# speechcatcher-asr/speechcatcher

Hardware: AMD Instinct MI355X
Metric: concurrent real-time streams (audio-seconds/s), de_xl dims, 640 ms (10240-sample) chunk steps, beam 10 CTC+attention (higher is better)
Workload: dtype f32

## Files before the change

### speechcatcher_amd/csrc/common.h

```cpp
#pragma once
#include <hip/hip_runtime.h>
#include <stdint.h>
#include <stdio.h>
#include <math.h>

#include "../../include/scasr.h"

#define SC_LOGZERO (-10000000000.0f)

void sc_set_error(const char *fmt, ...);

const char *sc_hook(const char *name);

__attribute__((visibility("hidden"))) int allow_large_lds(const void *fn, size_t need, size_t max_bytes, const char *what);

#define SC_CHECK_ARG(cond, msg)      \
  do {                               \
    if (!(cond)) {                   \
      sc_set_error("%s: %s", __func__, msg); \
      return SC_ERR_ARG;             \
    }                                \
  } while (0)

#define SC_CHECK_LAUNCH()                                              \
  do {                                                                 \
    hipError_t e__ = hipGetLastError();                                \
    if (e__ != hipSuccess) {                                           \
      sc_set_error("%s: launch failed: %s", __func__, hipGetErrorString(e__)); \
      return SC_ERR_LAUNCH;                                            \
    }                                                                  \
  } while (0)

__host__ __device__ static inline int cdiv(int a, int b) { return (a + b - 1) / b; }

#define SC_TRY(call) do { rc = (call); if (rc != SC_OK) return rc; } while (0)

struct ProfScope {
  bool on; hipEvent_t a, b; hipStream_t st;
  ProfScope(bool on_, hipEvent_t a_, hipEvent_t b_, hipStream_t st_) : on(on_), a(a_), b(b_), st(st_) {}
  ProfScope(const ProfScope &) = delete;
  __attribute__((visibility("hidden"))) ~ProfScope() {
    if (on) { (void)hipEventDestroy(a); (void)hipEventDestroy(b); }
  }
};
ProfScope sc_prof_begin(hipStream_t st);
void sc_prof_end(ProfScope &p, int kind, double flops, double bytes);

int sc_decode_step_form(const sc_search *sb);
int sc_gemm_colblocks(const float *A, const int32_t *a_rows, int lda, const float *W, const float *bias, float *C,
                      const int32_t *c_rows, int ldc, int M, int N, int K, int ncb, long cb_stride, int flags, void *stream);

int sc_dec_layer_hpw(const sc_search &sb);
int sc_dec_layer_stream_form(const sc_search &sb);
int sc_dec_layer_split_ffn(const sc_search &sb);

int sc_launch_reduce_ln_proj(const float *part, int npart, int part_M, const float *b2, const float *Xin, float *Xout,
                             const int32_t *rows, int M, int D, const float *ln_g, const float *ln_b, float ln_eps,
                             float *XN, const float *Wq, const float *bq, float *Q, int N, hipStream_t st,
                             int by_row = 0, int half_mode = 0);

struct ScHandoff { const int32_t *blkinfo; int R; float *state; int layer; };
int sc_ffn_ln_handoff(const float *XN, int M, int D, int F, const void *W1, const float *b1, const void *W2, const float *b2,
                      float *X, int w_form, const ScHandoff &ho, void *stream);

template <int CTRL>
__device__ __forceinline__ float dpp_mov(float v) {
  return __int_as_float(__builtin_amdgcn_update_dpp(0, __float_as_int(v), CTRL, 0xF, 0xF, true));
}
#define SC_DPP_XOR1 0xB1
#define SC_DPP_XOR2 0x4E
#define SC_DPP_HALF_MIRROR 0x141
#define SC_DPP_ROR4 0x124
#define SC_DPP_ROR8 0x128
#define SC_DPP_ROW_MIRROR 0x140

template <int LPR>
__device__ __forceinline__ float group_sum(float v) {
  v += dpp_mov<SC_DPP_XOR1>(v);
  v += dpp_mov<SC_DPP_XOR2>(v);
  if (LPR >= 8) v += dpp_mov<SC_DPP_HALF_MIRROR>(v);
  if (LPR == 16) v += dpp_mov<SC_DPP_ROW_MIRROR>(v);
  return v;
}

__device__ __forceinline__ float sc_lane(float v, int lane) {
  return __int_as_float(__builtin_amdgcn_readlane(__float_as_int(v), lane));
}
__device__ __forceinline__ float wave_max(float v) {
  v = fmaxf(v, dpp_mov<SC_DPP_XOR1>(v));
  v = fmaxf(v, dpp_mov<SC_DPP_XOR2>(v));
  v = fmaxf(v, dpp_mov<SC_DPP_HALF_MIRROR>(v));
  v = fmaxf(v, dpp_mov<SC_DPP_ROW_MIRROR>(v));
  return fmaxf(fmaxf(sc_lane(v, 0), sc_lane(v, 16)), fmaxf(sc_lane(v, 32), sc_lane(v, 48)));
}
__device__ __forceinline__ float wave_sum(float v) {
  v += dpp_mov<SC_DPP_XOR1>(v);
  v += dpp_mov<SC_DPP_XOR2>(v);
  v += dpp_mov<SC_DPP_HALF_MIRROR>(v);
  v += dpp_mov<SC_DPP_ROW_MIRROR>(v);
  return (sc_lane(v, 0) + sc_lane(v, 16)) + (sc_lane(v, 32) + sc_lane(v, 48));
}

#define SC_LOG2E 1.4426950408889634f
#define SC_LN2 0.6931471805599453f
__device__ __forceinline__ float sc_exp_neg(float x) {
  return __builtin_amdgcn_exp2f(x * SC_LOG2E);
}
__device__ __forceinline__ float sc_max_raw(float a, float b) {
  float m;
  asm("v_max_f32 %0, %1, %2" : "=v"(m) : "v"(a), "v"(b));
  return m;
}
__device__ __forceinline__ float lse2(float a, float b) {
  const float m = sc_max_raw(a, b);
  return m + SC_LN2 * __builtin_amdgcn_logf(1.f + sc_exp_neg(-fabsf(a - b)));
}

__device__ __forceinline__ float4 sc_add4(const float4 &a, const float4 &b) {
  return make_float4(a.x + b.x, a.y + b.y, a.z + b.z, a.w + b.w);
}
__device__ __forceinline__ float4 sc_tree4(const float4 &a, const float4 &b, const float4 &c, const float4 &d) {
  return sc_add4(sc_add4(a, b), sc_add4(c, d));
}
__device__ __forceinline__ float4 sc_tree8(const float4 (&v)[8]) {
  return sc_add4(sc_tree4(v[0], v[1], v[2], v[3]), sc_tree4(v[4], v[5], v[6], v[7]));
}
__device__ __forceinline__ float sc_tree8f(const float (&v)[8]) {
  return ((v[0] + v[1]) + (v[2] + v[3])) + ((v[4] + v[5]) + (v[6] + v[7]));
}
__device__ __forceinline__ float4 sc_seq4(const float4 &a, const float4 &b, const float4 &c, const float4 &d) {
  return sc_add4(sc_add4(sc_add4(a, b), c), d);
// ... 63 lines not shown
```

### speechcatcher_amd/csrc/search.hip

```cpp
#include "common.h"
#include "attn.h"
#include <mutex>
#include <unordered_map>

#define CTRL(s, f) sb.ctrl[(s) * 8 + (f)]
#define SC_CTC_T(s) (CTRL(s, SC_C_TCTC) > 0 ? CTRL(s, SC_C_TCTC) : CTRL(s, SC_C_T))

#define YSEQ(pp, s, h) (sb.yseq + (((long)(pp) * sb.S + (s)) * sb.W + (h)) * sb.LCAP)
#define XPOS(pp, s, h) (sb.xpos + (((long)(pp) * sb.S + (s)) * sb.W + (h)) * sb.LCAP)
#define ANC(pp, s) (sb.anc + ((long)(pp) * sb.S + (s)) * sb.LCAP * sb.W)
#define CTCR(pp, s) (sb.ctc_r + ((long)(pp) * sb.S + (s)) * sb.TCAP * 2 * sb.W)
#define CTCRS(pp, s) (sb.ctc_rs + ((long)(pp) * sb.S + (s)) * sb.TCAP * sb.W)

__global__ void ctc_extend_state_kernel(sc_search sb) {
  const int s = blockIdx.x, h = threadIdx.x;
  if (!CTRL(s, SC_C_ACTIVE) || !CTRL(s, SC_C_HAS)) return;
  const int T = CTRL(s, SC_C_T), told = CTRL(s, SC_C_TOLD), nh = CTRL(s, SC_C_NHYP);
  if (h >= nh || told >= T) return;
  float *r = CTCR(CTRL(s, SC_C_CUR), s);
  float *rs = CTCRS(CTRL(s, SC_C_CUR), s);
  const float *x = sb.ctcx + (long)s * sb.TCAP * sb.V;
  const int t0 = told < 1 ? 1 : told;
  float rb = r[((long)(t0 - 1) * 2 + 1) * sb.W + h];
  for (int t = t0; t < T; ++t) {
// ... 1069 lines not shown
          dst_rs[(long)t * W + i] = lse2(SC_LOGZERO, SC_LOGZERO);
        }
        if (start - 1 < t1) {
          dst[((long)(start - 1) * 2) * W + i] = r_n;
          dst[((long)(start - 1) * 2 + 1) * W + i] = r_b;
          dst_rs[(long)(start - 1) * W + i] = lse2(r_n, r_b);
        }
        t_lo = start;
      } else {
        r_n = ck[((long)(j - 1) * 2) * WK + e];
        r_b = ck[((long)(j - 1) * 2 + 1) * WK + e];
        t_lo = t0;
      }
      t_hi = t1;
    }
    if (t_lo >= t_hi) continue;
    float cum = 0.f;
    if (!has)
      for (int t = 0; t < t_lo; ++t) cum += xblk[t];
    for (int tb = t_lo & ~(SC_CTC_CK - 1); tb < t_hi; tb += SC_CTC_CK) {
      float xc[SC_CTC_CK], xb[SC_CTC_CK], pn[SC_CTC_CK], pb[SC_CTC_CK];
#pragma unroll
      for (int q = 0; q < SC_CTC_CK / 4; ++q) {
        const int t4 = min(tb + 4 * q, tct - 4);
        const float4 c4 = *reinterpret_cast<const float4 *>(xcol + t4), b4 = *reinterpret_cast<const float4 *>(xblk + t4);
        xc[4 * q] = c4.x; xc[4 * q + 1] = c4.y; xc[4 * q + 2] = c4.z; xc[4 * q + 3] = c4.w;
        xb[4 * q] = b4.x; xb[4 * q + 1] = b4.y; xb[4 * q + 2] = b4.z; xb[4 * q + 3] = b4.w;
      }
#pragma unroll
      for (int q = 0; q < SC_CTC_CK; ++q) {
        const int tp = min(max(tb + q - 1, 0), T - 1);
        pn[q] = has ? rsp[(long)tp * W + h] : 0.f;
        pb[q] = has ? rp[((long)tp * 2 + 1) * W + h] : 0.f;
      }
#pragma unroll
      for (int q = 0; q < SC_CTC_CK; ++q) {
        const int t = tb + q;
        if (t >= t_lo && t < t_hi) {
          float phi;
          ctc_frame(r_n, r_b, has ? pn[q] : cum, has ? pb[q] : cum, same, xc[q], xb[q], phi);
          dst[((long)t * 2) * W + i] = r_n;
          dst[((long)t * 2 + 1) * W + i] = r_b;
          dst_rs[(long)t * W + i] = lse2(r_n, r_b);
          if (!has) cum += xb[q];
        }
      }
    }
  }
}

extern "C" int sc_ctc_gather_state_split(const sc_search *sbp, int split_min, void *stream) {
  SC_CHECK_ARG(sbp, "null");
  SC_CHECK_ARG(sbp->ctcxT && sbp->tct >= 4, "the state rebuild needs the column-major table copy (sc_search.ctcxT)");
  int gx = cdiv(ctc_tck(sbp->TCAP) * sbp->W, 256);
  if (gx > 16) gx = 16;
  const int eff = ctc_split_min_ok(sbp->TCAP, split_min), last = scan_split_last(sbp);
  if (last >= 0 && last != eff) {
    sc_set_error("sc_ctc_gather_state_split: the last prefix scan of this batch ran with split_min = %d, the rebuild was asked for %d - "
                 "streams split over T leave segment states, not checkpoints: pass the scan's value (sc_ctc_gather_state() = 0)", last, eff);
    return SC_ERR_ARG;
  }
  ctc_gather_state_kernel<<<dim3(gx, sbp->S), 256, 0, (hipStream_t)stream>>>(*sbp, eff);
  SC_CHECK_LAUNCH();
  return SC_OK;
}

extern "C" int sc_ctc_gather_state(const sc_search *sbp, void *stream) { return sc_ctc_gather_state_split(sbp, 0, stream); }

static bool dec_fused_ok(const sc_search &sb) {
  if (const char *e = sc_hook("SC_DEC_FUSED"))
    return atoi(e) != 0 && sc_dec_layer_fused_supported(sb.d, sb.H, sb.W, sb.F) && sb.ph1 && sb.out_w_q;
  if (const char *e = sc_hook("SC_FUSED_MAX"))
    if ((sb.rowmap ? sb.n_rows : sb.S * sb.W) > atoi(e) && sc_dec_layer_hpw(sb) < 2) return false;
  return sc_dec_layer_fused_supported(sb.d, sb.H, sb.W, sb.F) && sb.ph1 && sb.ph2 && sb.ffn_part &&
         sb.max_ffn_part >= 1 && sb.out_w_q && sb.V % sb.d == 0 && sb.layers && sb.layers[0].wqkv_pp &&
         sb.layers[0].wq_pp && sb.layers[0].wo_pp && sb.layers[0].w1_p;
}

int sc_decode_step_form(const sc_search *sbp) { return dec_fused_ok(*sbp) ? (sc_dec_layer_stream_form(*sbp) ? 2 : 1) : 0; }

extern "C" int sc_decode_step(const sc_search *sbp, void *stream) { return sc_decode_step_ex(sbp, 0, stream); }

extern "C" int sc_decode_step_ex(const sc_search *sbp, int scan_split_min, void *stream) {
  SC_CHECK_ARG(sbp, "null");
  const sc_search &sb = *sbp;
  const int n = sb.rowmap ? sb.n_rows : sb.S * sb.W;
  int rc;
  if (dec_fused_ok(sb) && sc_dec_layer_stream_form(sb)) {
    float *xa = sb.dx, *xb = sb.dxn;
    int npart = 0;
    for (int li = 0; li < sb.n_layers; ++li) {
      SC_TRY(sc_dec_layer_stream(sbp, li, xa, xb, sb.dq, sb.ffn_part, npart, stream));
      SC_TRY(sc_dec_layer_ffn_xn(sbp, li, sb.dq, sb.ffn_part, sb.max_ffn_part, &npart, stream));
      float *t = xa; xa = xb; xb = t;
    }
    SC_TRY(sc_dec_output_logits(sbp, xa, xb, sb.ffn_part, npart, stream));
  } else if (dec_fused_ok(sb)) {
    float *xa = sb.dx, *xb = sb.dxn;
    int npart = 0;
    for (int li = 0; li < sb.n_layers; ++li) {
      SC_TRY(sc_dec_layer_self(sbp, li, xa, xb, sb.ffn_part, npart, stream));
      SC_TRY(sc_dec_layer_cross(sbp, li, xb, xa, stream));
      if (sc_dec_layer_split_ffn(sb)) {
        SC_TRY(sc_dec_layer_reduce_ln(sbp, li, xa, xb, sb.dq, stream));
        SC_TRY(sc_dec_layer_ffn_xn(sbp, li, sb.dq, sb.ffn_part, sb.max_ffn_part, &npart, stream));
      } else
      SC_TRY(sc_dec_layer_ffn(sbp, li, xa, xb, sb.ffn_part, sb.max_ffn_part, &npart, stream));
      float *t = xa; xa = xb; xb = t;
    }
    SC_TRY(sc_dec_output_logits(sbp, xa, xb, sb.ffn_part, npart, stream));
  } else {
  SC_TRY(sc_dec_embed(sbp, stream));
  bool logits_done = false;
  SC_TRY(decoder_layers_impl(sbp, stream, true, &logits_done));
  if (!logits_done)
    SC_TRY(sc_gemm(sb.dxn, sb.rowmap, sb.d, sb.out_w, sb.out_b, sb.logits, sb.rowmap, sb.V, n, sb.V, sb.d, 0, 0, stream));
  }
  SC_TRY(sc_logsoftmax_topk(sbp, stream));
  const bool use_ctc = sb.w_ctc > 0.f;
  if (use_ctc) SC_TRY(sc_ctc_prefix_scan_split(sbp, scan_split_min, stream));
  SC_TRY(sc_fuse_topw(sbp, stream));
  SC_TRY(sc_beam_prune(sbp, stream));
  if (use_ctc) SC_TRY(sc_ctc_gather_state_split(sbp, scan_split_min, stream));
  return SC_OK;
}
```

### speechcatcher_amd/csrc/streams.hip

```cpp
#include <algorithm>
#include <array>
#include <chrono>
#include <cmath>
#include <cstdarg>
#include <cstring>
#include <deque>
#include <map>
#include <memory>
#include <new>
#include <string>
#include <vector>

#include "common.h"
#include "resample.h"

namespace {

#define HIP_TRY(call)                                                              \
  do {                                                                             \
    hipError_t e__ = (call);                                                       \
    if (e__ != hipSuccess) {                                                       \
      sc_set_error("%s: %s failed: %s", __func__, #call, hipGetErrorString(e__));  \
      return SC_ERR_LAUNCH;                                                        \
    }                                                                              \
// ... 63 lines not shown
  int T_proj = 0, T_projkv = 0;
  long n_steps_total = 0;
  int T_hyp = 0;
  int rs_tab = -1, rs_par = 0;
  long rs_in = 0, rs_out = 0;
};

struct Blk { int T; bool fin; long gen; long job; };

struct Run {
  bool inblk = false, live = false, took = false, pvalid = false, has = false, hasp = false, fin = false;
  int cur = 0, L = 1, nhyp = 1, nhp = 1, pidx = 0, T = 0, Tc = 0, out = 0;
  long nsteps = 0;
  long job = 0;
};

struct ActVal {
  bool ready = true;
  long gen = 0;
  int32_t v[6] = {0, 0, 0, -1, -1, 0};
  int T = 0;
};

struct Job {
  bool open = false;
  int has_out = 0;
  int fault = 0;
  long seq = 0;
  bool fin = false;
  bool dropped = false;
  bool started = false;
  ActVal act;
};

struct Snap {
  bool valid = false, reported = false;
  long seq = 0;
  int L = 1, nhyp = 0;
  int T = 0;
};

template <typename T>
int dalloc(T **p, size_t n) {
  const size_t bytes = std::max<size_t>(n, 1) * sizeof(T);
  HIP_TRY(hipMalloc((void **)p, bytes));
  HIP_TRY(hipMemset(*p, 0, bytes));
  return SC_OK;
}

}

struct EncPlan {
  std::vector<int32_t> conv_jobs, a_rows, lin_dst, feat_src, feat_dst, blk_jobs, sjobs, emit_src, emit_dst, sub_src,
      sub_dst;
  struct Short { int s, ubase, U, pe_pos, dst_T; };
  std::vector<Short> shorts;
  int n_conv = 0, max_t1 = 0;
};

struct EncGroup {
  long gen = 0;
  bool launched = false, features = false;
  bool open = false;
  bool deferred = false;
  int slot = 0;
  int stage_slot = -1;
  std::vector<long long> copy_jobs;
  std::vector<sc_rs_job> rs_jobs;
  size_t stage_floats = 0;
  std::vector<int32_t> fe_jobs;
  int n_fe = 0, max_keep = 0;
  EncPlan P;
  std::vector<int32_t> ctc_rows, kv_src, kv_dst;
  struct ActSpan { int s, t0, t1; long epoch; bool restart; };
  std::vector<ActSpan> act;
  bool same_rows = true;
  std::vector<int> streams;
  bool empty() const { return !n_fe && !P.n_conv; }
};

constexpr int N_ARENA = 8;
constexpr int N_STAGE = 4;
constexpr int N_RING = 4;

struct sc_streams {
  sc_engine *eng = nullptr;
  sc_config cfg{};
  int S = 0, W = 0, K = 0, TCAP = 0, LCAP = 0, FCAP = 0, UCAP = 0, max_feat_new = 0, max_t1 = 0, max_t2 = 0,
      max_blocks = 0, max_chunk = 0, max_length = 500;
  long PCAP = 0;
  bool use_bbd = false, strict = true;
  hipStream_t stream = nullptr;
  hipStream_t stream_enc = nullptr, es = nullptr;
  hipEvent_t ev_iter[2] = {nullptr, nullptr};
  int32_t *ring_dev = nullptr;
  int32_t *rm_host[2] = {nullptr, nullptr};
  int rm_idx = 0;
  bool rm_dirty = false;
  int scan_split_min = 1024, scan_split_streams = 0;
  bool scan_long = false;
  int step_split_min() const { return (scan_long && (scan_split_streams <= 0 || n_rows_step <= scan_split_streams * W)) ? scan_split_min : 0; }
  int graph_key() const { return n_rows_step * 2 + (step_split_min() > 0 ? 1 : 0); }
  int enc_start_thr = 0;
  int enc_batch_min = 0;
  int gemm_flags = 0;
  void *ws = nullptr, *ws_enc = nullptr;
  std::vector<void *> owned, owned_host;
  float *pcm = nullptr, *featbuf = nullptr, *subbuf = nullptr, *prev_addin = nullptr, *past_ctx = nullptr, *enc = nullptr,
        *c1 = nullptr, *c2 = nullptr, *xblk = nullptr, *ws_xn = nullptr, *ws_qkv = nullptr, *ws_att = nullptr,
        *ws_ffh = nullptr;
  int32_t *jobs_ctx = nullptr, *ctrlmap = nullptr;
  float *kv_stage = nullptr;
  int kv_stage_rows = 0;
  sc_search sb{};
  int32_t *ctrlmap_host = nullptr, *flags_host = nullptr;
  int32_t *arena_host = nullptr, *arena_dev = nullptr;
  size_t slot_cap = 0, arena_off = 0;
  int cur_slot = 0;
  hipEvent_t ev_group[N_ARENA] = {nullptr};
  long slot_gen[N_ARENA] = {0};
  int32_t *bs_host = nullptr, *bs_dev = nullptr;
  size_t bs_cap = 0;
  int bs_i = 0;
  float *stage_host = nullptr, *stage_dev = nullptr;
  size_t stage_cap = 0;
  hipEvent_t ev_stage[N_STAGE] = {nullptr};
  bool stage_busy[N_STAGE] = {false};
  int stage_next = 0;
  long long *cjobs_host = nullptr, *cjobs_dev = nullptr;
  sc_rs_job *rsjobs_host = nullptr, *rsjobs_dev = nullptr;
  float *rs_hist = nullptr;
  sc_rs_tabs rs_tabs{};
  int rs_rate[SC_RS_MAX_TABS] = {0};
  int n_rs_tabs = 0;
  int32_t *pack_dev = nullptr, *pack_host = nullptr, *pjobs_host = nullptr, *pjobs_dev = nullptr;
  size_t pack_cap = 0;
  char *al_dev = nullptr;
  size_t al_cap = 0;
  bool act_on = false;
  double act_thr = 0.8;
  int32_t *act_state = nullptr;
  double *act_track = nullptr;
  sc_ctc_activity_job *act_jobs_host = nullptr, *act_jobs_dev = nullptr;
  int32_t *act_out_host = nullptr, *act_out_dev = nullptr;
  std::vector<ActVal> act_known;
  std::vector<ActVal> act_rep;
  std::vector<long> act_pending;
  std::vector<long> act_epoch;
  std::vector<char> act_fresh;
  std::vector<St> st;
  std::vector<Run> run;
  std::vector<std::deque<Blk>> bq;
  std::vector<Job> job;
  std::vector<std::deque<Job>> ahead;
  std::vector<long> job_seq;
  int queue_depth = 1;
  std::vector<Snap> snap;
  std::vector<long> done_at;
  long done_counter = 0;
  int32_t *snap_yseq = nullptr, *snap_xpos = nullptr;
  double *snap_score = nullptr;
  hipEvent_t ev_snap = nullptr;
  std::vector<std::string> fault_msg;
  std::vector<long> enc_gen;
  std::deque<EncGroup *> groups;
  long gen_next = 1, gen_done = 0, gen_ordered = 0;
  int n_open = 0;
  long iter = 0;
  bool inflight = false;
  std::vector<int> tick_active;
  std::chrono::steady_clock::time_point tick_t0, tick_t1;
  hipStream_t stream_rb = nullptr;
  bool poisoned = false;
  std::vector<int> rowmap_key;
  int row_bucket = 1, n_rows_step = 0;
  bool decode_prepared = false;
  std::map<int, hipGraphExec_t> dec_graphs;
  std::map<std::vector<long>, hipGraphExec_t> enc_graphs;
  long dec_steps = 0, dec_blocks = 0, enc_calls = 0, xattn_rows[3] = {0, 0, 0};
  long sattn_pos[3] = {0, 0, 0};
  unsigned long long *stat_rows = nullptr;
  double t_launch = 0, t_wait = 0;
  double t_bucket[17] = {0};
  long n_bucket[17] = {0};
  bool use_graphs = true;
  long n_enc_captures = 0;
  double t_enc_capture = 0;

  ~sc_streams() {
    for (auto &g : dec_graphs) (void)hipGraphExecDestroy(g.second);
    for (auto &g : enc_graphs) (void)hipGraphExecDestroy(g.second);
    if (stream) (void)sc_set_stream_workspace(stream, nullptr, 0);
    if (stream_enc) {
      (void)sc_set_stream_workspace(stream_enc, nullptr, 0);
      (void)hipStreamDestroy(stream_enc);
    }
    for (int i = 0; i < 2; ++i)
      if (ev_iter[i]) (void)hipEventDestroy(ev_iter[i]);
    for (int i = 0; i < N_ARENA; ++i)
      if (ev_group[i]) (void)hipEventDestroy(ev_group[i]);
    for (int i = 0; i < N_STAGE; ++i)
      if (ev_stage[i]) (void)hipEventDestroy(ev_stage[i]);
    if (ev_snap) (void)hipEventDestroy(ev_snap);
    for (EncGroup *g : groups) delete g;
    for (void *p : owned) (void)hipFree(p);
    for (void *p : owned_host) (void)hipHostFree(p);
    if (stream_rb) (void)hipStreamDestroy(stream_rb);
    if (stream) (void)hipStreamDestroy(stream);
    if (al_dev) (void)hipFree(al_dev);
  }

  template <typename T>
  int alloc(T **p, size_t n) {
    RC_TRY(dalloc(p, n));
    owned.push_back(*p);
    return SC_OK;
  }
  template <typename T>
  int halloc(T **p, size_t n) {
    HIP_TRY(hipHostMalloc((void **)p, std::max<size_t>(n, 1) * sizeof(T)));
    owned_host.push_back(*p);
    memset(*p, 0, std::max<size_t>(n, 1) * sizeof(T));
    return SC_OK;
  }
  int32_t *ctrl_host() { return ctrlmap_host; }
  int32_t *rowmap_host() { return rm_host[rm_idx]; }

  int itensor(const std::vector<int32_t> &a, const int32_t **out) {
    const size_t n = a.size();
    if (arena_off + n > slot_cap) {
      sc_set_error("job-table arena exhausted (%zu + %zu of %zu entries)", arena_off, n, slot_cap);
      return SC_ERR_ARG;
    }
    const size_t off = (size_t)cur_slot * slot_cap + arena_off;
    arena_off += (n + 63) & ~size_t(63);
    if (n) {
      memcpy(arena_host + off, a.data(), n * sizeof(int32_t));
      HIP_TRY(hipMemcpyAsync(arena_dev + off, arena_host + off, n * sizeof(int32_t), hipMemcpyHostToDevice, es));
    }
    *out = arena_dev + off;
    return SC_OK;
  }
};


namespace {

constexpr int F_ANY_EOS = 1, F_BEST_EOS = 2, F_ALL_EOS = 4, F_REPEAT = 8;

__global__ void init_hyp_kernel(sc_search sb, int s) {
  const size_t o = ((size_t)0 * sb.S + s) * sb.W + 0;
  sb.yseq[o * sb.LCAP] = sb.sos;
  sb.xpos[o * sb.LCAP] = 0;
  sb.anc[((size_t)0 * sb.S + s) * sb.LCAP * sb.W] = 0;
  sb.score[o] = 0.0;
  sb.sc_dec[o] = 0.0;
  sb.sc_ctc[o] = 0.0;
}

__global__ __launch_bounds__(256) void scatter_f32_kernel(const float *__restrict__ src, float *__restrict__ dst,
                                                          const long long *__restrict__ jobs) {
  const long long so = jobs[blockIdx.y * 3], dof = jobs[blockIdx.y * 3 + 1], n = jobs[blockIdx.y * 3 + 2];
  for (long long i = (long long)blockIdx.x * 256 + threadIdx.x; i < n; i += (long long)gridDim.x * 256) dst[dof + i] = src[so + i];
}

void launch_scatter(const float *src, float *dst, const long long *jobs_dev, int nj, long long mx, hipStream_t st) {
  dim3 grid((unsigned)std::min<long long>(64, (std::max<long long>(mx, 1) + 1023) / 1024), nj);
  scatter_f32_kernel<<<grid, 256, 0, st>>>(src, dst, jobs_dev);
}

__global__ __launch_bounds__(128) void pack_hyps_kernel(sc_search sb, const int32_t *__restrict__ jobs, int32_t *__restrict__ out,
                                                        const int32_t *__restrict__ snap_yseq, const int32_t *__restrict__ snap_xpos,
                                                        const double *__restrict__ snap_score) {
  const int32_t *j = jobs + (size_t)blockIdx.x * 4;
  const size_t row = (size_t)j[0];
  const int L = j[1];
  const bool snap = j[3] != 0;
  int32_t *o = out + (size_t)j[2];
  const int32_t *ys = (snap ? snap_yseq : sb.yseq) + row * sb.LCAP, *xp = (snap ? snap_xpos : sb.xpos) + row * sb.LCAP;
  for (int i = threadIdx.x; i < L; i += 128) {
    o[i] = ys[i];
    o[L + i] = xp[i];
  }
  if (threadIdx.x == 0) {
    double *sc = (double *)(o + ((2 * L + 1) & ~1));
    sc[0] = snap ? snap_score[row * 3] : sb.score[row];
    sc[1] = snap ? snap_score[row * 3 + 1] : sb.sc_dec[row];
    sc[2] = snap ? snap_score[row * 3 + 2] : sb.sc_ctc[row];
  }
}

struct SnapArgs { int n; int s[32], cur[32], L[32], nhyp[32]; };
__global__ __launch_bounds__(128) void snapshot_hyps_kernel(sc_search sb, SnapArgs a, int32_t *__restrict__ snap_yseq,
                                                            int32_t *__restrict__ snap_xpos, double *__restrict__ snap_score) {
  const int e = blockIdx.x, h = blockIdx.y;
  if (h >= a.nhyp[e]) return;
  const size_t src = ((size_t)a.cur[e] * sb.S + a.s[e]) * sb.W + h, dst = (size_t)a.s[e] * sb.W + h;
  for (int i = threadIdx.x; i < a.L[e]; i += 128) {
    snap_yseq[dst * sb.LCAP + i] = sb.yseq[src * sb.LCAP + i];
    snap_xpos[dst * sb.LCAP + i] = sb.xpos[src * sb.LCAP + i];
  }
  if (threadIdx.x == 0) {
    snap_score[dst * 3] = sb.score[src];
    snap_score[dst * 3 + 1] = sb.sc_dec[src];
    snap_score[dst * 3 + 2] = sb.sc_ctc[src];
  }
}

// ... 254 lines not shown
                      c.ln_eps, b->es));
  return SC_OK;
}

int encode_launch(sc_streams *b, EncPlan &P) {
  const sc_config &c = b->cfg;
  sc_engine *e = b->eng;
  const int d = c.d_model, F1 = c.conv_freq1, F2 = c.conv_freq2, R = c.block_size + 2;
  b->enc_calls++;
  const int32_t *cj, *ar, *ld;
  RC_TRY(b->itensor(P.conv_jobs, &cj));
  RC_TRY(sc_conv1(b->featbuf, c.n_mels, cj, P.n_conv, P.max_t1, e->f("conv1_w"), e->f("conv1_b"), d, b->c1, b->es));
  RC_TRY(b->itensor(P.a_rows, &ar));
  RC_TRY(sc_gemm(b->c1, ar, d, e->f("conv2_w"), e->f("conv2_b"), b->c2, nullptr, d, (int)P.a_rows.size(), d, 9 * d,
                 SC_GEMM_RELU | b->gemm_flags, F1, b->es));
  RC_TRY(b->itensor(P.lin_dst, &ld));
  RC_TRY(sc_gemm(b->c2, nullptr, F2 * d, e->f("sub_out_w"), e->f("sub_out_b"), b->subbuf, ld, d, (int)P.lin_dst.size(), d,
                 F2 * d, b->gemm_flags, 0, b->es));
  if (!P.feat_src.empty()) {
    const int32_t *a, *z;
    RC_TRY(b->itensor(P.feat_src, &a));
    RC_TRY(b->itensor(P.feat_dst, &z));
    RC_TRY(sc_copy_rows(b->featbuf, a, b->featbuf, z, (int)P.feat_src.size(), c.n_mels, b->es));
  }
  const int nbk = (int)P.blk_jobs.size() / 6, ns = (int)P.sjobs.size() / 5;
  if (nbk > 0) {
    if (nbk > b->max_blocks) {
      sc_set_error("sc_push: too many encoder blocks in one call");
      return SC_ERR_ARG;
    }
    const int32_t *bj, *ja;
    RC_TRY(b->itensor(P.blk_jobs, &bj));
    RC_TRY(sc_block_pack(b->subbuf, bj, nbk, R, e->f("pe"), d, b->xblk, b->es));
    std::vector<int32_t> j_add(ns * 4), j_ctx(ns * 4);
    for (int i = 0; i < ns; ++i) {
      const int32_t *sj = &P.sjobs[i * 5];
      j_add[i * 4 + 0] = sj[0]; j_add[i * 4 + 1] = sj[1]; j_add[i * 4 + 2] = sj[2]; j_add[i * 4 + 3] = sj[3];
      j_ctx[i * 4 + 0] = sj[0]; j_ctx[i * 4 + 1] = sj[1]; j_ctx[i * 4 + 2] = sj[2] * c.enc_layers; j_ctx[i * 4 + 3] = sj[4];
    }
    RC_TRY(b->itensor(j_add, &ja));
    RC_TRY(sc_ctx_handoff(b->xblk, R, ja, ns, b->prev_addin, 0, d, b->es));
    const int32_t *jc;
    RC_TRY(b->itensor(j_ctx, &jc));
    HIP_TRY(hipMemcpyAsync(b->jobs_ctx, jc, j_ctx.size() * sizeof(int32_t), hipMemcpyDeviceToDevice, b->es));
    RC_TRY(enc_layers_launch(b, nbk, R, true, b->jobs_ctx, ns));
  }
  if (!P.emit_src.empty()) {
    const int32_t *a, *z;
    RC_TRY(b->itensor(P.emit_src, &a));
    RC_TRY(b->itensor(P.emit_dst, &z));
    RC_TRY(sc_layernorm(b->xblk, a, d, b->enc, z, d, (int)P.emit_src.size(), d, e->f("enc_norm_g"), e->f("enc_norm_b"),
                        c.ln_eps, b->es));
  }
  for (auto &sh : P.shorts) RC_TRY(encode_short(b, sh));
  if (!P.sub_src.empty()) {
    const int32_t *a, *z;
    RC_TRY(b->itensor(P.sub_src, &a));
    RC_TRY(b->itensor(P.sub_dst, &z));
    RC_TRY(sc_copy_rows(b->subbuf, a, b->subbuf, z, (int)P.sub_src.size(), d, b->es));
  }
  return SC_OK;
}

void set_rowmap(sc_streams *b, const std::vector<int> &active) {
  const int S = b->S, W = b->W;
  const int na = (int)active.size();
  const int nb = std::min(S, (na + b->row_bucket - 1) / b->row_bucket * b->row_bucket);
  if (active != b->rowmap_key) {
    b->rowmap_key = active;
    b->rm_idx ^= 1;
    b->rm_dirty = true;
    int32_t *rm = b->rowmap_host();
    std::vector<char> isact(S, 0);
    for (int s : active) isact[s] = 1;
    int k = 0;
    for (int pass = 1; pass >= 0; --pass)
      for (int s = 0; s < S; ++s)
        if (isact[s] == pass)
          for (int h = 0; h < W; ++h) rm[k++] = s * W + h;
  }
  b->n_rows_step = nb * W;
}

int decode_step_launch(sc_streams *b) {
  b->sb.n_rows = b->n_rows_step;
  b->sb.flags = b->ring_dev;
  auto step = [&]() { return sc_decode_step_ex(&b->sb, b->step_split_min(), b->stream); };
  if (!b->use_graphs) return step();
  auto it = b->dec_graphs.find(b->graph_key());
  if (it == b->dec_graphs.end()) {
    RC_TRY(step());
    RC_TRY(sc_graph_capture_begin(b->stream));
    const int rc = step();
    void *g = nullptr;
    const int rc2 = sc_graph_capture_end(b->stream, &g);
    if (rc != SC_OK) return rc;
    if (rc2 != SC_OK) return rc2;
    b->dec_graphs[b->graph_key()] = (hipGraphExec_t)g;
    return SC_OK;
  }
  return sc_graph_launch(it->second, b->stream);
}

int prepare_decode(sc_streams *b) {
  memset(b->ctrl_host(), 0, (size_t)b->S * 8 * sizeof(int32_t));
  HIP_TRY(hipMemcpyAsync(b->ctrlmap, b->ctrlmap_host, (size_t)b->S * 8 * sizeof(int32_t), hipMemcpyHostToDevice, b->stream));
  const int keep = b->n_rows_step;
  for (int nb = b->row_bucket; nb < b->S + b->row_bucket; nb += b->row_bucket) {
    b->n_rows_step = std::min(nb, b->S) * b->W;
    if (!b->dec_graphs.count(b->graph_key())) RC_TRY(decode_step_launch(b));
  }
  b->n_rows_step = keep;
  HIP_TRY(hipStreamSynchronize(b->stream));
  return SC_OK;
}

int retire_groups(sc_streams *b) {
  while (!b->groups.empty()) {
    EncGroup *g = b->groups.front();
    if (!g->launched) break;
    const hipError_t q = hipEventQuery(b->ev_group[g->slot]);
    if (q == hipErrorNotReady) { (void)hipGetLastError(); break; }
    if (q != hipSuccess) {
      sc_set_error("encoder group %ld failed: %s", g->gen, hipGetErrorString(q));
      return SC_ERR_LAUNCH;
    }
    for (size_t i = 0; i < g->act.size(); ++i) {
      const EncGroup::ActSpan &sp = g->act[i];
      if (sp.epoch != b->act_epoch[sp.s]) continue;
      ActVal &k = b->act_known[sp.s];
      k.ready = true;
      k.gen = g->gen;
      k.T = sp.t1;
      memcpy(k.v, b->act_out_host + ((size_t)g->slot * b->S + i) * 6, sizeof k.v);
      auto fill = [&](ActVal &a) {
        if (!a.ready && a.gen == g->gen) a = k;
      };
      fill(b->job[sp.s].act);
      for (Job &j : b->ahead[sp.s]) fill(j.act);
      fill(b->act_rep[sp.s]);
    }
    b->gen_done = g->gen;
    b->slot_gen[g->slot] = 0;
    b->groups.pop_front();
    delete g;
  }
  return SC_OK;
}

int launch_pending_groups(sc_streams *b, long upto = -1);
int wait_group(sc_streams *b, long gen) {
  if (gen <= b->gen_done) return SC_OK;
  RC_TRY(launch_pending_groups(b, gen));
  const int slot = (int)(gen % N_ARENA);
  HIP_TRY(hipEventSynchronize(b->ev_group[slot]));
  return retire_groups(b);
}

int project_rows(sc_streams *b, EncGroup &g) {
  const sc_config &c = b->cfg;
  sc_engine *e = b->eng;
  const int d = c.d_model, Ld = c.dec_layers, V = c.vocab_size;
  const int32_t *ar = nullptr;
  if (!g.ctc_rows.empty()) {
    RC_TRY(b->itensor(g.ctc_rows, &ar));
    RC_TRY(sc_gemm(b->enc, ar, d, e->f("ctc_w"), e->f("ctc_b"), const_cast<float *>(b->sb.ctcx), ar, V, (int)g.ctc_rows.size(),
                   V, d, b->gemm_flags, 0, b->es));
    if (!g.act.empty()) {
      const int n = (int)g.act.size();
      if (n > b->S) {
        sc_set_error("activity: %d spans in a group of a batch of %d streams (internal error)", n, b->S);
        return SC_ERR_ARG;
      }
      const size_t o = (size_t)g.slot * b->S;
      for (int i = 0; i < n; ++i) {
        const EncGroup::ActSpan &sp = g.act[i];
        sc_ctc_activity_job &j = b->act_jobs_host[o + i];
        j.table = b->sb.ctcx + (size_t)sp.s * b->TCAP * V;
        j.state = b->act_state + (size_t)sp.s * 6;
        j.track = b->act_track + (size_t)sp.s * b->TCAP;
        j.state_after = b->act_out_dev + (o + i) * 6;
        j.stride = V;
        j.thr = b->act_thr;
        j.V = V; j.blank = c.blank_id; j.t0 = sp.t0; j.t1 = sp.t1;
        j.restart = sp.restart ? 1 : 0;
        j.reserved = 0;
      }
      HIP_TRY(hipMemcpyAsync(b->act_jobs_dev + o, b->act_jobs_host + o, (size_t)n * sizeof(sc_ctc_activity_job),
                             hipMemcpyHostToDevice, b->es));
// ... 217 lines not shown
  for (int s : starts) {
    const Blk k = b->bq[s].front();
    b->bq[s].pop_front();
    St &x = b->st[s];
    Run &r = b->run[s];
    r = Run();
    r.inblk = r.live = true;
    r.T = k.T; r.fin = k.fin; r.job = k.job;
    r.cur = x.cur; r.L = x.L; r.nhyp = x.nhyp; r.has = x.has_ctc; r.pidx = x.process_idx; r.pvalid = x.prev_valid;
    const int told = x.T_ctc;
    r.Tc = std::max(k.T, told);
    if (k.T > told && told == 0)
      for (int t = 0; t < k.T && n_lsm < (int)(b->bs_cap - (size_t)S * 8); ++t) lsm[n_lsm++] = s * b->TCAP + t;
    int32_t *c = ctrl0 + s * 8;
    c[0] = 1; c[1] = r.cur; c[2] = r.fin; c[3] = r.Tc; c[4] = r.L; c[5] = r.nhyp; c[6] = r.has; c[7] = told;
    x.T_ctc = r.Tc;
    x.T_kv = std::max(k.T, x.T_kv);
    x.output_index = 0;
    r.nhp = r.nhyp; r.hasp = r.has;
    b->dec_blocks++;
  }
  HIP_TRY(hipMemcpyAsync(b->ctrlmap, ctrl0, (size_t)S * 8 * sizeof(int32_t), hipMemcpyHostToDevice, b->stream));
  if (n_lsm) {
    int32_t *ld = b->bs_dev + (size_t)b->bs_i * b->bs_cap;
    HIP_TRY(hipMemcpyAsync(ld, lsm, (size_t)n_lsm * sizeof(int32_t), hipMemcpyHostToDevice, b->stream));
    RC_TRY(sc_log_softmax_rows(const_cast<float *>(b->sb.ctcx), ld, n_lsm, b->cfg.vocab_size, b->stream));
  }
  RC_TRY(sc_ctc_extend_state(&b->sb, b->stream));
  return SC_OK;
}

int tick_collect(sc_streams *b);
int tick_issue(sc_streams *b, bool *progress) {
  const int S = b->S, W = b->W, Ld = b->cfg.dec_layers;
  *progress = false;
  if (b->inflight) RC_TRY(tick_collect(b));
  RC_TRY(retire_groups(b));
  RC_TRY(snapshot_completed(b));
  RC_TRY(start_blocks(b));
  {
    long need = 0;
    for (int s = 0; s < S; ++s)
      if (!b->run[s].inblk && !b->bq[s].empty()) need = std::max(need, b->bq[s].front().gen);
    long upto = -1;
    for (EncGroup *g : b->groups)
      if (!g->launched && g->deferred && g->gen <= need) upto = g->gen;
    if (upto >= 0) RC_TRY(launch_pending_groups(b, upto));
  }
  std::vector<int> &active = b->tick_active;
  active.clear();
  for (int s = 0; s < S; ++s) {
    Run &r = b->run[s];
    if (!r.inblk) continue;
    const bool act = r.live && r.pidx < b->max_length;
    if (act && r.L + 1 > b->LCAP) {
      fault_stream(b, s, SC_ERR_CAPACITY, "max_tokens exceeded");
      *progress = true;
      continue;
    }
    if (!act) {
      finish_block(b, s);
      *progress = true;
      continue;
    }
    active.push_back(s);
  }
  if (active.empty()) {
    if (*progress) return SC_OK;
    long need = 0;
    for (int s = 0; s < S; ++s)
      if (!b->run[s].inblk && !b->bq[s].empty() && (need == 0 || b->bq[s].front().gen < need)) need = b->bq[s].front().gen;
    if (need > std::max(b->gen_done, b->gen_ordered)) {
      RC_TRY(launch_pending_groups(b, need));
      if (b->stream_enc) HIP_TRY(hipStreamWaitEvent(b->stream, b->ev_group[need % N_ARENA], 0));
      b->gen_ordered = std::max(b->gen_ordered, need);
      *progress = true;
    }
    return SC_OK;
  }
  *progress = true;
  b->tick_t0 = std::chrono::steady_clock::now();
  set_rowmap(b, active);
  b->scan_long = false;
  int32_t *ctrl = b->ctrl_host();
  memset(ctrl, 0, (size_t)S * 8 * sizeof(int32_t));
  for (int s : active) {
    const Run &r = b->run[s];
    if (b->scan_split_min > 0 && r.Tc - std::max(r.L - 1, 1) >= b->scan_split_min) b->scan_long = true;
    int32_t *c = ctrl + s * 8;
    c[0] = 1; c[1] = r.cur; c[2] = r.fin; c[3] = r.T; c[4] = r.L; c[5] = r.nhyp; c[6] = r.has; c[7] = r.Tc;
  }
  if ((int)active.size() <= b->enc_start_thr)
    for (EncGroup *g : b->groups)
      if (!g->launched && !g->open) RC_TRY(launch_group(b, g));
  if (b->rm_dirty) {
    memcpy(b->ctrlmap_host + S * 8, b->rm_host[b->rm_idx], (size_t)S * W * sizeof(int32_t));
    HIP_TRY(hipMemcpyAsync(b->ctrlmap, b->ctrlmap_host, (size_t)(S * 8 + S * W) * sizeof(int32_t), hipMemcpyHostToDevice, b->stream));
    b->rm_dirty = false;
  } else {
    HIP_TRY(hipMemcpyAsync(b->ctrlmap, b->ctrlmap_host, (size_t)S * 8 * sizeof(int32_t), hipMemcpyHostToDevice, b->stream));
  }
  RC_TRY(decode_step_launch(b));
  HIP_TRY(hipEventRecord(b->ev_iter[b->iter & 1], b->stream));
  const int form = sc_decode_step_form(&b->sb);
  for (int s : active) {
    b->xattn_rows[form] += (long)b->run[s].T * Ld;
    b->sattn_pos[form] += (long)b->run[s].L * Ld;
  }
  b->tick_t1 = std::chrono::steady_clock::now();
  b->inflight = true;
  return SC_OK;
}

int tick_collect(sc_streams *b) {
  if (!b->inflight) return SC_OK;
  const int S = b->S, W = b->W;
  b->inflight = false;
  const auto tpw = std::chrono::steady_clock::now();
  HIP_TRY(hipEventSynchronize(b->ev_iter[b->iter & 1]));
  const auto tp2 = std::chrono::steady_clock::now();
  b->iter++;
  b->dec_steps++;
  b->t_launch += std::chrono::duration<double>(b->tick_t1 - b->tick_t0).count();
  b->t_wait += std::chrono::duration<double>(tp2 - tpw).count();
  {
    const int bk = std::min(16, (int)((long)b->n_rows_step * 16 / std::max(1, S * W)));
    b->t_bucket[bk] += std::chrono::duration<double>(tp2 - b->tick_t0).count();
    b->n_bucket[bk] += 1;
  }
  for (int s : b->tick_active) {
    Run &r = b->run[s];
    const bool kv_full = b->flags_host[S + s] != 0;
    b->flags_host[S + s] = 0;
    const int f = b->flags_host[s];
    const bool f_any = f & F_ANY_EOS, f_best = f & F_BEST_EOS, f_all = f & F_ALL_EOS, f_rep = f & F_REPEAT;
    r.out += 1;
    r.nsteps += 1;
    const bool stop_eos = f_any && (!r.fin || f_best);
    const bool stop_bbd = b->use_bbd && !stop_eos && f_rep && !r.fin;
    const bool stop_all = !stop_eos && !stop_bbd && f_all && r.fin;
    const bool accept = !(stop_eos || stop_bbd || stop_all);
    const bool take = stop_eos || stop_all || accept;
    if (kv_full && take && !(!accept && r.pidx > 1 && r.pvalid)) {
      fault_stream(b, s, SC_ERR_CAPACITY, "self-attention K|V pool exhausted (kv_pool_rows / max_tokens)");
      continue;
    }
    if (stop_bbd) r.out -= 1;
    if (take) {
      r.nhp = r.nhyp;
      r.hasp = r.has;
      r.cur = 1 - r.cur;
      r.L += 1;
      r.nhyp = std::min(W, r.nhyp * W);
      r.has = true;
    }
    if (stop_eos || stop_all) r.took = true;
    r.live = accept;
    if (accept) {
      r.pvalid = true;
      r.pidx += 1;
    }
    if (!(r.live && r.pidx < b->max_length)) finish_block(b, s);
  }
  return SC_OK;
}

int engine_tick(sc_streams *b, bool *progress) {
  RC_TRY(tick_issue(b, progress));
  return tick_collect(b);
}

inline bool chunk_decoded(const sc_streams *b, int s) {
  const long q = b->job[s].seq;
  return !(b->run[s].inblk && b->run[s].job <= q) && (b->bq[s].empty() || b->bq[s].front().job > q);
}
inline bool chunk_complete(const sc_streams *b, int s) {
  const Job &j = b->job[s];
  if (!j.open) return false;
  if (j.fault != 0) return true;
  if (!chunk_decoded(b, s)) return false;
  return b->queue_depth <= 1 || (b->snap[s].valid && b->snap[s].seq == j.seq);
}

struct Chunk { int s; const float *host; long n; bool fin; int pos; };

inline long st_gen(const sc_streams *b, int s) { return b->enc_gen[s] > b->gen_done ? b->enc_gen[s] : 0; }
// ... 564 lines not shown
  A(sb.ctc_r, (size_t)2 * S * b->TCAP * 2 * W);
  A(sb.ctc_rs, (size_t)2 * S * b->TCAP * W);
  A(sb.ctc_s, 2 * n);
  A(sb.ctc_rnew, (size_t)S * ((b->TCAP + 15) / 16) * 2 * W * K);
  A(sb.dx, n * d); A(sb.dxn, n * d); A(sb.dqkv, n * 3 * d); A(sb.datt, n * d); A(sb.dq, n * d); A(sb.dffh, n * F);
  A(sb.logits, n * V); A(sb.logp, n * V);
  A(sb.pre_ids, n * K); A(sb.psi, n * K); A(sb.psi_eos, n);
  A(sb.cand_score, n * W); A(sb.cand_tok, n * W); A(sb.cand_ctc, n * W);
  A(sb.sel, n * 2);
  A(b->stat_rows, 3);
  sb.stat_rows = b->stat_rows;
  if (sc_dec_layer_fused_supported(d, c.dec_heads, W, F) && V % d == 0 && e->dec[0].wqkv_pp && e->f("out_w_q", false)) {
    A(sb.ph1, n * c.dec_heads * d);
    A(sb.ph2, n * c.dec_heads * d);
    A(sb.ffn_part, (size_t)(F / 128) * n * d);
    sb.max_ffn_part = F / 128;
  }
  if (rc == SC_OK && hipMalloc(&b->ws, (size_t)128 << 20) != hipSuccess) rc = SC_ERR_LAUNCH;
  if (rc == SC_OK) b->owned.push_back(b->ws);
#undef A
  if (rc != SC_OK) {
    sc_set_error("sc_streams_create: device allocation failed");
    delete b;
    return rc;
  }
  sb.ctrl = b->ctrlmap;
  sb.rowmap = b->ctrlmap + S * 8;
  sb.n_rows = S * W;
  sb.embed = e->f("embed"); sb.pe = e->f("pe"); sb.dec_norm_g = e->f("dec_norm_g"); sb.dec_norm_b = e->f("dec_norm_b");
  sb.out_w = e->f("out_w"); sb.out_b = e->f("out_b"); sb.out_w_q = e->f("out_w_q", false);
  sb.out_w_qh = nullptr;
  sb.act_half = 0;
  if (sb.kv_half && e->f("out_w_qh", false) && !e->dec.empty() && e->dec[0].wqkv_pph && e->dec[0].wq_pph && e->dec[0].wo_pph &&
      e->dec[0].wo2_pph && sb.ph1) {
    sb.out_w_qh = e->f("out_w_qh", false);
    sb.act_half = 1 | 2;
    if (const char *ah = sc_hook("SC_ACT_HALF")) sb.act_half = atoi(ah) & 7;
  }
  sb.layers = e->dec.data();
  (void)sc_set_stream_workspace(b->stream, b->ws, (size_t)128 << 20);
  b->es = b->stream;
  {
    b->enc_start_thr = S < 16 ? S : std::max(1, (int)((long)S * 7 / 100));
  }
  {
    const hipError_t er = hipStreamCreateWithPriority(&b->stream_enc, hipStreamNonBlocking, 0);
    if (er == hipSuccess && hipMalloc(&b->ws_enc, (size_t)128 << 20) == hipSuccess) {
      b->owned.push_back(b->ws_enc);
      (void)sc_set_stream_workspace(b->stream_enc, b->ws_enc, (size_t)128 << 20);
    } else {
      (void)hipGetLastError();
      if (b->stream_enc) (void)hipStreamDestroy(b->stream_enc);
      b->stream_enc = nullptr;
    }
  }
  const size_t cm = ((size_t)S * 8 + n) * sizeof(int32_t);
  bool ok = b->halloc(&b->ctrlmap_host, (size_t)S * 8 + n) == SC_OK && b->halloc(&b->flags_host, (size_t)S * 2) == SC_OK &&
            b->halloc(&b->rm_host[0], n) == SC_OK && b->halloc(&b->rm_host[1], n) == SC_OK &&
            b->halloc(&b->arena_host, b->slot_cap * N_ARENA) == SC_OK && b->halloc(&b->bs_host, b->bs_cap * N_RING) == SC_OK &&
            b->halloc(&b->stage_host, b->stage_cap * N_STAGE) == SC_OK && b->halloc(&b->pack_host, b->pack_cap) == SC_OK &&
            b->halloc(&b->pjobs_host, n * 4) == SC_OK && b->halloc(&b->cjobs_host, (size_t)N_STAGE * S * 3) == SC_OK &&
            b->halloc(&b->rsjobs_host, (size_t)N_STAGE * S) == SC_OK;
  for (int i = 0; i < 2 && ok; ++i) ok = hipEventCreateWithFlags(&b->ev_iter[i], hipEventDisableTiming) == hipSuccess;
  for (int i = 0; i < N_ARENA && ok; ++i) ok = hipEventCreateWithFlags(&b->ev_group[i], hipEventDisableTiming) == hipSuccess;
  for (int i = 0; i < N_STAGE && ok; ++i) ok = hipEventCreateWithFlags(&b->ev_stage[i], hipEventDisableTiming) == hipSuccess;
  if (!ok) {
    sc_set_error("sc_streams_create: pinned host allocation failed");
    delete b;
    return SC_ERR_LAUNCH;
  }
  memset(b->flags_host, 0, (size_t)S * 8);
  {
    void *dv = nullptr;
    if (hipHostGetDevicePointer(&dv, b->flags_host, 0) != hipSuccess || !dv) {
      sc_set_error("sc_streams_create: pinned flags are not device-accessible");
      delete b;
      return SC_ERR_LAUNCH;
    }
    b->ring_dev = (int32_t *)dv;
    sb.flags = b->ring_dev;
    sb.kvflags = b->ring_dev + S;
  }
  if (const char *sp = sc_hook("SC_SCAN_SPLIT_MIN")) b->scan_split_min = atoi(sp);
  memset(b->ctrlmap_host, 0, cm);
  for (size_t i = 0; i < n; ++i) b->rm_host[0][i] = b->rm_host[1][i] = (int32_t)i;
  (void)hipMemcpy(b->ctrlmap, b->ctrlmap_host, (size_t)S * 8 * sizeof(int32_t), hipMemcpyHostToDevice);
  (void)hipMemcpy(b->ctrlmap + S * 8, b->rm_host[0], n * sizeof(int32_t), hipMemcpyHostToDevice);
  b->rowmap_key.resize(S);
  for (int s = 0; s < S; ++s) b->rowmap_key[s] = s;
  b->enc_batch_min = std::max(1, S / 2);
  b->gemm_flags = (!b->eng->enc.empty() && b->eng->enc[0].wqkv_s) ? SC_GEMM_SPLIT16 : 0;
  b->row_bucket = std::max(1, S / 32);
  b->n_rows_step = S * W;
  b->st.assign(S, St());
  b->run.assign(S, Run());
  b->bq.assign(S, std::deque<Blk>());
  b->job.assign(S, Job());
  b->ahead.assign(S, std::deque<Job>());
  b->job_seq.assign(S, 0);
  b->snap.assign(S, Snap());
  b->done_at.assign(S, 0);
  b->fault_msg.assign(S, std::string());
  b->enc_gen.assign(S, 0);
  for (int s = 0; s < S; ++s) init_hyp(b, s);
  *out = b;
  return SC_OK;
  SC_API_END
}

extern "C" void sc_streams_destroy(sc_streams *b) {
  if (b) {
    (void)hipStreamSynchronize(b->stream);
    if (b->stream_enc) (void)hipStreamSynchronize(b->stream_enc);
    delete b;
  }
}

extern "C" int sc_reset(sc_streams *b, int stream) {
  SC_CHECK_ARG(b && stream >= 0 && stream < b->S, "stream out of range");
  SC_CHECK_ARG(!b->job[stream].open, "the stream has a chunk outstanding (sc_poll reports it first)");
  reset_stream(b, stream);
  return SC_OK;
}

extern "C" int sc_stream_set_input_rate(sc_streams *b, int stream, int rate) {
  SC_CHECK_ARG(b && stream >= 0 && stream < b->S, "stream out of range");
  SC_API_BEGIN
  const St &cur = b->st[stream];
  SC_CHECK_ARG(!b->job[stream].open && b->ahead[stream].empty(), "the stream has a chunk outstanding (sc_poll reports it first)");
  SC_CHECK_ARG(cur.pcm_end == 0 && !cur.fe_started && !cur.enc_started && !cur.started && cur.rs_in == 0,
               "the stream has buffered audio since its last reset (sc_reset first)");
  int L, M, Wc;
  if (!sc_rs_params(rate, &L, &M, &Wc)) {
    sc_set_error("sc_stream_set_input_rate: unsupported input rate %d (supported: 8000..48000 Hz with 16000 / gcd(rate, 16000) <= 640)", rate);
    return SC_ERR_ARG;
  }
  int t = -1;
  if (rate != 16000) {
    for (int i = 0; i < b->n_rs_tabs; ++i)
      if (b->rs_rate[i] == rate) t = i;
    if (t < 0) {
      SC_CHECK_ARG(b->n_rs_tabs < SC_RS_MAX_TABS, "at most 8 distinct input rates per sc_streams");
      HIP_TRY(hipSetDevice(b->eng->device));
      std::vector<float> host((size_t)L * 2 * Wc);
      RC_TRY(sc_resample_design(rate, nullptr, nullptr, nullptr, host.data()));
      float *dev = nullptr;
      RC_TRY(b->alloc(&dev, host.size()));
      HIP_TRY(hipMemcpy(dev, host.data(), host.size() * sizeof(float), hipMemcpyHostToDevice));
      t = b->n_rs_tabs++;
      b->rs_rate[t] = rate;
      b->rs_tabs.coef[t] = dev;
      b->rs_tabs.L[t] = L; b->rs_tabs.M[t] = M; b->rs_tabs.Wc[t] = Wc;
    }
  }
  b->st[stream].rs_tab = t;
  return SC_OK;
  SC_API_END
}

extern "C" int sc_stream_input_rate(const sc_streams *b, int stream) {
  SC_CHECK_ARG(b && stream >= 0 && stream < b->S, "stream out of range");
  return b->st[stream].rs_tab < 0 ? 16000 : b->rs_rate[b->st[stream].rs_tab];
}

extern "C" int sc_stage_bench(int rate, int n_jobs, int n_in, int iters, double *ms) {
  SC_CHECK_ARG(n_jobs > 0 && n_jobs <= 4096 && n_in > 0 && n_in <= (1 << 20) && iters > 0 && ms, "bad arguments");
// ... 743 lines not shown
```

Measured before the change: 4109.

## Publish decode control via mapped host image and split CTC gather tail

Replaces the per-step host-to-device memcpy of the control block and rowmap with a double-buffered pinned, device-mapped control image. A small fetch kernel inside the decode graph copies it into device memory. The decode step is split into a head graph and a separate CTC-state gather tail graph, and the iteration event is recorded after the head, so the host can collect results before the gather finishes. This cuts copy-API overhead and host wait latency per step, but relies on host/device memory-ordering through a coherent mapped buffer and a sequence header.

```diff
diff --git a/speechcatcher_amd/csrc/common.h b/speechcatcher_amd/csrc/common.h
--- a/speechcatcher_amd/csrc/common.h
+++ b/speechcatcher_amd/csrc/common.h
@@ -47,6 +47,8 @@
 void sc_prof_end(ProfScope &p, int kind, double flops, double bytes);
 
 int sc_decode_step_form(const sc_search *sb);
+int sc_decode_step_head(const sc_search *sb, int scan_split_min, void *stream);
+int sc_decode_step_finish(const sc_search *sb, int scan_split_min, void *stream);
 int sc_gemm_colblocks(const float *A, const int32_t *a_rows, int lda, const float *W, const float *bias, float *C,
                       const int32_t *c_rows, int ldc, int M, int N, int K, int ncb, long cb_stride, int flags, void *stream);
 
diff --git a/speechcatcher_amd/csrc/search.hip b/speechcatcher_amd/csrc/search.hip
--- a/speechcatcher_amd/csrc/search.hip
+++ b/speechcatcher_amd/csrc/search.hip
@@ -1175,6 +1175,18 @@
 extern "C" int sc_decode_step(const sc_search *sbp, void *stream) { return sc_decode_step_ex(sbp, 0, stream); }
 
 extern "C" int sc_decode_step_ex(const sc_search *sbp, int scan_split_min, void *stream) {
+  int rc;
+  SC_TRY(sc_decode_step_head(sbp, scan_split_min, stream));
+  return sc_decode_step_finish(sbp, scan_split_min, stream);
+}
+
+int sc_decode_step_finish(const sc_search *sbp, int scan_split_min, void *stream) {
+  SC_CHECK_ARG(sbp, "null");
+  if (sbp->w_ctc > 0.f) return sc_ctc_gather_state_split(sbp, scan_split_min, stream);
+  return SC_OK;
+}
+
+int sc_decode_step_head(const sc_search *sbp, int scan_split_min, void *stream) {
   SC_CHECK_ARG(sbp, "null");
   const sc_search &sb = *sbp;
   const int n = sb.rowmap ? sb.n_rows : sb.S * sb.W;
@@ -1214,6 +1226,5 @@
   if (use_ctc) SC_TRY(sc_ctc_prefix_scan_split(sbp, scan_split_min, stream));
   SC_TRY(sc_fuse_topw(sbp, stream));
   SC_TRY(sc_beam_prune(sbp, stream));
-  if (use_ctc) SC_TRY(sc_ctc_gather_state_split(sbp, scan_split_min, stream));
   return SC_OK;
 }
diff --git a/speechcatcher_amd/csrc/streams.hip b/speechcatcher_amd/csrc/streams.hip
--- a/speechcatcher_amd/csrc/streams.hip
+++ b/speechcatcher_amd/csrc/streams.hip
@@ -169,6 +169,7 @@
 constexpr int N_ARENA = 8;
 constexpr int N_STAGE = 4;
 constexpr int N_RING = 4;
+constexpr int FETCH_HDR = 64;
 
 struct sc_streams {
   sc_engine *eng = nullptr;
@@ -180,6 +181,10 @@
   hipStream_t stream = nullptr;
   hipStream_t stream_enc = nullptr, es = nullptr;
   hipEvent_t ev_iter[2] = {nullptr, nullptr};
+  bool step_boundary = true;
+  int32_t *fetch_host = nullptr, *fetch_dev = nullptr;
+  int fetch_par = 0;
+  unsigned fetch_seq = 0;
   int32_t *ring_dev = nullptr;
   int32_t *rm_host[2] = {nullptr, nullptr};
   int rm_idx = 0;
@@ -263,6 +268,7 @@
   int row_bucket = 1, n_rows_step = 0;
   bool decode_prepared = false;
   std::map<int, hipGraphExec_t> dec_graphs;
+  std::map<int, hipGraphExec_t> dec_tail_graphs;
   std::map<std::vector<long>, hipGraphExec_t> enc_graphs;
   long dec_steps = 0, dec_blocks = 0, enc_calls = 0, xattn_rows[3] = {0, 0, 0};
   long sattn_pos[3] = {0, 0, 0};
@@ -276,6 +282,7 @@
 
   ~sc_streams() {
     for (auto &g : dec_graphs) (void)hipGraphExecDestroy(g.second);
+    for (auto &g : dec_tail_graphs) (void)hipGraphExecDestroy(g.second);
     for (auto &g : enc_graphs) (void)hipGraphExecDestroy(g.second);
     if (stream) (void)sc_set_stream_workspace(stream, nullptr, 0);
     if (stream_enc) {
@@ -310,7 +317,10 @@
     memset(*p, 0, std::max<size_t>(n, 1) * sizeof(T));
     return SC_OK;
   }
-  int32_t *ctrl_host() { return ctrlmap_host; }
+  size_t fetch_image_ints() const { return (size_t)S * 8 + (size_t)S * W; }
+  int32_t *ctrl_host() {
+    return step_boundary ? fetch_host + FETCH_HDR + (size_t)fetch_par * fetch_image_ints() : ctrlmap_host;
+  }
   int32_t *rowmap_host() { return rm_host[rm_idx]; }
 
   int itensor(const std::vector<int32_t> &a, const int32_t **out) {
@@ -731,29 +741,89 @@
   b->n_rows_step = nb * W;
 }
 
+__global__ __launch_bounds__(256) void ctrl_fetch_kernel(const int32_t *img, int32_t *__restrict__ dst, int n_ctrl, int n_all) {
+  const int hdr = __hip_atomic_load(img, __ATOMIC_RELAXED, __HIP_MEMORY_SCOPE_SYSTEM);
+  const int i = blockIdx.x * 256 + threadIdx.x;
+  if (i >= n_all || (i >= n_ctrl && !(hdr & 2))) return;
+  dst[i] = __hip_atomic_load(img + FETCH_HDR + (size_t)(hdr & 1) * n_all + i, __ATOMIC_RELAXED, __HIP_MEMORY_SCOPE_SYSTEM);
+}
+
+int launch_ctrl_fetch(sc_streams *b) {
+  const int n_ctrl = b->S * 8, n_all = (int)b->fetch_image_ints();
+  ctrl_fetch_kernel<<<(n_all + 255) / 256, 256, 0, b->stream>>>(b->fetch_dev, b->ctrlmap, n_ctrl, n_all);
+  SC_CHECK_LAUNCH();
+  return SC_OK;
+}
+
+void publish_ctrl(sc_streams *b) {
+  const int dirty = b->rm_dirty ? 1 : 0;
+  if (dirty) memcpy(b->ctrl_host() + (size_t)b->S * 8, b->rm_host[b->rm_idx], (size_t)b->S * b->W * sizeof(int32_t));
+  b->rm_dirty = false;
+  const unsigned hdr = (++b->fetch_seq << 2) | (unsigned)(dirty << 1) | (unsigned)b->fetch_par;
+  __atomic_store_n(b->fetch_host, (int32_t)hdr, __ATOMIC_RELEASE);
+}
+
 int decode_step_launch(sc_streams *b) {
   b->sb.n_rows = b->n_rows_step;
   b->sb.flags = b->ring_dev;
-  auto step = [&]() { return sc_decode_step_ex(&b->sb, b->step_split_min(), b->stream); };
-  if (!b->use_graphs) return step();
-  auto it = b->dec_graphs.find(b->graph_key());
-  if (it == b->dec_graphs.end()) {
-    RC_TRY(step());
-    RC_TRY(sc_graph_capture_begin(b->stream));
-    const int rc = step();
-    void *g = nullptr;
-    const int rc2 = sc_graph_capture_end(b->stream, &g);
-    if (rc != SC_OK) return rc;
-    if (rc2 != SC_OK) return rc2;
-    b->dec_graphs[b->graph_key()] = (hipGraphExec_t)g;
+  const int split = b->step_split_min(), key = b->graph_key();
+  hipEvent_t ev = b->ev_iter[b->iter & 1];
+  if (!b->step_boundary) {
+    auto step = [&]() { return sc_decode_step_ex(&b->sb, split, b->stream); };
+    auto it = b->dec_graphs.find(key);
+    if (!b->use_graphs) {
+      RC_TRY(step());
+    } else if (it == b->dec_graphs.end()) {
+      RC_TRY(step());
+      RC_TRY(sc_graph_capture_begin(b->stream));
+      const int rc = step();
+      void *g = nullptr;
+      const int rc2 = sc_graph_capture_end(b->stream, &g);
+      if (rc != SC_OK) return rc;
+      if (rc2 != SC_OK) return rc2;
+      b->dec_graphs[key] = (hipGraphExec_t)g;
+    } else {
+      RC_TRY(sc_graph_launch(it->second, b->stream));
+    }
+    HIP_TRY(hipEventRecord(ev, b->stream));
     return SC_OK;
   }
-  return sc_graph_launch(it->second, b->stream);
+  const bool has_tail = b->sb.w_ctc > 0.f;
+  auto head = [&]() -> int {
+    RC_TRY(launch_ctrl_fetch(b));
+    return sc_decode_step_head(&b->sb, split, b->stream);
+  };
+  auto tail = [&]() { return sc_decode_step_finish(&b->sb, split, b->stream); };
+  auto it = b->dec_graphs.find(key);
+  if (!b->use_graphs || it == b->dec_graphs.end()) {
+    RC_TRY(head());
+    HIP_TRY(hipEventRecord(ev, b->stream));
+    RC_TRY(tail());
+    if (!b->use_graphs) return SC_OK;
+    auto capture = [&](auto &&what, std::map<int, hipGraphExec_t> &into) -> int {
+      RC_TRY(sc_graph_capture_begin(b->stream));
+      const int rc = what();
+      void *g = nullptr;
+      const int rc2 = sc_graph_capture_end(b->stream, &g);
+      if (rc != SC_OK) return rc;
+      if (rc2 != SC_OK) return rc2;
+      into[key] = (hipGraphExec_t)g;
+      return SC_OK;
+    };
+    RC_TRY(capture(head, b->dec_graphs));
+    if (has_tail) RC_TRY(capture(tail, b->dec_tail_graphs));
+    return SC_OK;
+  }
+  RC_TRY(sc_graph_launch(it->second, b->stream));
+  HIP_TRY(hipEventRecord(ev, b->stream));
+  if (has_tail) RC_TRY(sc_graph_launch(b->dec_tail_graphs.at(key), b->stream));
+  return SC_OK;
 }
 
 int prepare_decode(sc_streams *b) {
   memset(b->ctrl_host(), 0, (size_t)b->S * 8 * sizeof(int32_t));
-  HIP_TRY(hipMemcpyAsync(b->ctrlmap, b->ctrlmap_host, (size_t)b->S * 8 * sizeof(int32_t), hipMemcpyHostToDevice, b->stream));
+  if (b->step_boundary) publish_ctrl(b);
+  else HIP_TRY(hipMemcpyAsync(b->ctrlmap, b->ctrlmap_host, (size_t)b->S * 8 * sizeof(int32_t), hipMemcpyHostToDevice, b->stream));
   const int keep = b->n_rows_step;
   for (int nb = b->row_bucket; nb < b->S + b->row_bucket; nb += b->row_bucket) {
     b->n_rows_step = std::min(nb, b->S) * b->W;
@@ -1137,6 +1207,7 @@
   b->tick_t0 = std::chrono::steady_clock::now();
   set_rowmap(b, active);
   b->scan_long = false;
+  b->fetch_par ^= 1;
   int32_t *ctrl = b->ctrl_host();
   memset(ctrl, 0, (size_t)S * 8 * sizeof(int32_t));
   for (int s : active) {
@@ -1148,7 +1219,9 @@
   if ((int)active.size() <= b->enc_start_thr)
     for (EncGroup *g : b->groups)
       if (!g->launched && !g->open) RC_TRY(launch_group(b, g));
-  if (b->rm_dirty) {
+  if (b->step_boundary) {
+    publish_ctrl(b);
+  } else if (b->rm_dirty) {
     memcpy(b->ctrlmap_host + S * 8, b->rm_host[b->rm_idx], (size_t)S * W * sizeof(int32_t));
     HIP_TRY(hipMemcpyAsync(b->ctrlmap, b->ctrlmap_host, (size_t)(S * 8 + S * W) * sizeof(int32_t), hipMemcpyHostToDevice, b->stream));
     b->rm_dirty = false;
@@ -1156,7 +1229,6 @@
     HIP_TRY(hipMemcpyAsync(b->ctrlmap, b->ctrlmap_host, (size_t)S * 8 * sizeof(int32_t), hipMemcpyHostToDevice, b->stream));
   }
   RC_TRY(decode_step_launch(b));
-  HIP_TRY(hipEventRecord(b->ev_iter[b->iter & 1], b->stream));
   const int form = sc_decode_step_form(&b->sb);
   for (int s : active) {
     b->xattn_rows[form] += (long)b->run[s].T * Ld;
@@ -1887,6 +1959,20 @@
     sb.kvflags = b->ring_dev + S;
   }
   if (const char *sp = sc_hook("SC_SCAN_SPLIT_MIN")) b->scan_split_min = atoi(sp);
+  if (const char *sp = sc_hook("SC_STEP_BOUNDARY")) b->step_boundary = atoi(sp) != 0;
+  {
+    const size_t fi = FETCH_HDR + 2 * b->fetch_image_ints();
+    void *dv = nullptr;
+    if (hipHostMalloc((void **)&b->fetch_host, fi * sizeof(int32_t), hipHostMallocMapped | hipHostMallocCoherent) == hipSuccess)
+      b->owned_host.push_back(b->fetch_host);
+    if (!b->fetch_host || hipHostGetDevicePointer(&dv, b->fetch_host, 0) != hipSuccess || !dv) {
+      sc_set_error("sc_streams_create: the control image is not device-accessible");
+      delete b;
+      return SC_ERR_LAUNCH;
+    }
+    b->fetch_dev = (int32_t *)dv;
+    memset(b->fetch_host, 0, fi * sizeof(int32_t));
+  }
   memset(b->ctrlmap_host, 0, cm);
   for (size_t i = 0; i < n; ++i) b->rm_host[0][i] = b->rm_host[1][i] = (int32_t)i;
   (void)hipMemcpy(b->ctrlmap, b->ctrlmap_host, (size_t)S * 8 * sizeof(int32_t), hipMemcpyHostToDevice);
```

Measured after the change: 4076. No clear change (-0.8%).
